# AnnaUshnova/tinyrenderder

Hardware: AMD Instinct MI355X
Metric: triangles/sec (+ Mpixels/sec) at 4096x4096; achieved HBM GB/s vs peak (higher is better)
Workload: dtype f64

## Files before the change

tinyrenderder_amd/api.py:

```python
from __future__ import annotations

import ctypes as C
import os
import sys

import numpy as np

HERE = os.path.dirname(os.path.abspath(__file__))
LIB_PATH = os.path.join(HERE, "libtrgl.so")

FLAT, GOURAUD, PHONG, EYE, CHECKER = 0, 1, 2, 3, 4
VARY = {FLAT: 0, GOURAUD: 3, PHONG: 24, EYE: 24, CHECKER: 0}
SHADER_USER_FIRST, MAX_USER_SHADERS, MAX_USER_VARY = 64, 32, 64
SHADER_MAY_DISCARD = 1
SHADER_READS_DEST = 4
SHADER_NO_DEPTH_WRITE = 8


def shader_flags(may_discard=False, reads_dest=False, depth_write=True) -> int:
    return ((SHADER_MAY_DISCARD if may_discard else 0) | (SHADER_READS_DEST if reads_dest else 0)
            | (0 if depth_write else SHADER_NO_DEPTH_WRITE))
MAX_USER_VERTEX_SHADERS = 32
MEM_HOST, MEM_DEVICE = 0, 1
PHASE_SETUP, PHASE_BIN, PHASE_RASTER, PHASE_TOTAL, PHASE_RASTER_KERNEL = 0, 1, 2, 3, 4
# ... 131 lines not shown
    L.trgl_draw.argtypes = [vp, C.c_int, C.POINTER(Uniforms), C.c_void_p, C.c_void_p, C.c_void_p, C.c_uint64, C.c_int]
    L.trgl_flush.argtypes = [vp]
    L.trgl_flush_begin.argtypes = [vp]
    L.trgl_flush_end.argtypes = [vp]
    L.trgl_sync.argtypes = [vp]
    L.trgl_read_framebuffer.argtypes = [vp, C.c_void_p]
    L.trgl_write_framebuffer.argtypes = [vp, C.c_void_p]
    L.trgl_read_zbuffer.argtypes = [vp, C.c_void_p]
    L.trgl_write_zbuffer.argtypes = [vp, C.c_void_p]
    L.trgl_get_stats.argtypes = [vp, C.POINTER(Stats)]
    L.trgl_reset_stats.argtypes = [vp]
    L.trgl_format_stats.argtypes = [C.POINTER(Stats), C.c_char_p, C.c_size_t]
    for name in ("trgl_framebuffer_device_ptr", "trgl_zbuffer_device_ptr", "trgl_stream"):
        getattr(L, name).argtypes = [vp]; getattr(L, name).restype = C.c_void_p
    L.trgl_set_stream.argtypes = [vp, C.c_void_p, C.c_int]
    L.trgl_set_profiling.argtypes = [vp, C.c_int]
    L.trgl_get_phase_ms.argtypes = [vp, dp, u64p]
    L.trgl_reset_phase_ms.argtypes = [vp]
    L.trgl_get_last_flush_info.argtypes = [vp, u64p, u64p, u64p]
    if hasattr(L, "trgl_debug_read"):
        L.trgl_debug_read.argtypes = [vp, C.c_int, C.c_void_p, C.c_size_t, C.POINTER(C.c_size_t)]
    if hasattr(L, "trgl_debug_binning"):
        L.trgl_debug_binning.argtypes = [vp, C.c_int, C.c_uint32, C.c_uint32, C.POINTER(C.c_int), C.POINTER(C.c_int)]
    L.trgl_selftest_division.argtypes = [vp, C.c_uint64, C.c_uint64, u64p]
    L.trgl_selftest_sampler.argtypes = [vp, C.c_int, C.c_void_p, C.c_uint64, C.c_void_p]
    L.trgl_draw_indexed.argtypes = [vp, C.c_int, C.POINTER(Uniforms), dp, C.c_void_p, C.c_int, C.c_uint64, C.c_void_p, C.c_uint64, C.c_int]
    L.trgl_ssao_defaults.argtypes = [C.POINTER(SsaoParams)]
    L.trgl_ssao_defaults.restype = None
    L.trgl_postprocess.argtypes = [vp, C.POINTER(SsaoParams), C.c_void_p, C.c_void_p, C.c_void_p]
    L.trgl_obj_load.argtypes = [C.c_char_p, C.POINTER(C.POINTER(C.c_double)), u64p, C.POINTER(C.POINTER(C.c_uint32)), u64p]
    L.trgl_obj_free.argtypes = [C.POINTER(C.c_double), C.POINTER(C.c_uint32)]
    L.trgl_obj_free.restype = None
    L.trgl_tga_max_size.argtypes = [C.c_int, C.c_int, C.c_int]
    L.trgl_tga_max_size.restype = C.c_size_t
    L.trgl_tga_encode.argtypes = [C.c_void_p, C.c_int, C.c_int, C.c_int, C.c_int, C.c_int, C.c_void_p, C.POINTER(C.c_size_t)]
    L.trgl_tga_info.argtypes = [C.c_void_p, C.c_size_t, C.POINTER(C.c_int), C.POINTER(C.c_int), C.POINTER(C.c_int)]
    L.trgl_tga_decode.argtypes = [C.c_void_p, C.c_size_t, C.c_void_p]
    L.trgl_gather.argtypes = [vp, C.c_void_p, C.c_int, C.c_int, C.c_int]
    L.trgl_rccl_unique_id.argtypes = [C.c_void_p]
    L.trgl_rccl_comm_create.argtypes = [C.c_void_p, C.c_int, C.c_int, C.c_int, C.POINTER(C.c_void_p)]
    L.trgl_rccl_comm_destroy.argtypes = [C.c_void_p]
    L.trgl_shader_compile.argtypes = [C.c_char_p, C.c_int, C.c_char_p, C.c_size_t]
    L.trgl_register_shader.argtypes = [vp, C.c_char_p, C.c_int, C.POINTER(C.c_int)]
    L.trgl_shader_compile_ex.argtypes = [C.c_char_p, C.c_int, C.c_uint32, C.c_char_p, C.c_size_t]
    L.trgl_register_shader_ex.argtypes = [vp, C.c_char_p, C.c_int, C.c_uint32, C.POINTER(C.c_int)]
    L.trgl_vertex_shader_compile.argtypes = [C.c_char_p, C.c_int, C.c_char_p, C.c_size_t]
# ... 1092 lines not shown
        self._chk(self.L.trgl_reset_phase_ms(self.h))

    def selftest_division(self, samples: int, seed: int = 1) -> int:
        bad = C.c_uint64()
        self._chk(self.L.trgl_selftest_division(self.h, samples, seed, C.byref(bad)))
        return bad.value

    def selftest_sampler(self, slot: int, uv) -> np.ndarray:
        uv = np.ascontiguousarray(uv, np.float64).reshape(-1, 2)
        out = np.zeros((uv.shape[0], 5), np.uint8)
        self._chk(self.L.trgl_selftest_sampler(self.h, slot, uv.ctypes.data, uv.shape[0], out.ctypes.data))
        return out

    def last_flush_info(self):
        a, b, c = C.c_uint64(), C.c_uint64(), C.c_uint64()
        self._chk(self.L.trgl_get_last_flush_info(self.h, C.byref(a), C.byref(b), C.byref(c)))
        return dict(triangles=a.value, pairs=b.value, tiles=c.value)

    def debug_binning(self, mode=None, S=0, G=0):
        d, f = C.c_int(), C.c_int()
        self._chk(self.L.trgl_debug_binning(self.h, -1 if mode is None else mode, S, G, C.byref(d), C.byref(f)))
        return dict(direct=bool(d.value), fell_back=bool(f.value))

    def _debug_read(self, what, dtype):
        need = C.c_size_t()
        self._chk(self.L.trgl_debug_read(self.h, what, None, 0, C.byref(need)))
        out = np.zeros(need.value // np.dtype(dtype).itemsize, dtype)
        if need.value:
            self._chk(self.L.trgl_debug_read(self.h, what, out.ctypes.data, out.nbytes, None))
        return out

    def debug_snapshot(self):
        info = dict(zip(DBG_INFO_FIELDS, (int(v) for v in self._debug_read(DBG_INFO, np.int64))))
        return dict(info=info, recs=self._debug_read(DBG_RECS, TRI_REC), cnt=self._debug_read(DBG_CNT, np.uint32),
                    tilebox=self._debug_read(DBG_TILEBOX, np.uint32).reshape(-1, 2), vals=self._debug_read(DBG_VALS, np.uint32),
                    bmask=self._debug_read(DBG_BMASK, np.uint16), tile_start=self._debug_read(DBG_TILE_START, np.uint32),
                    tile_end=self._debug_read(DBG_TILE_END, np.uint32))
```

tinyrenderder_amd/csrc/kernels_bin.hip:

```cpp
#include <hip/hip_runtime.h>
#include "trgl_device.h"
#include "launch.h"
#include "device_util.h"

namespace {

__device__ __forceinline__ double dmin3(double a, double b, double c) { double m = a; if (b < m) m = b; if (c < m) m = c; return m; }
__device__ __forceinline__ double dmax3(double a, double b, double c) { double m = a; if (m < b) m = b; if (m < c) m = c; return m; }
using trgl_dev::dot4; using trgl_dev::wave_incl_scan; using trgl_dev::block_excl_scan;

__device__ __forceinline__ int wave_min_i(int v) {
    for (int o = 32; o; o >>= 1) { int t = __shfl_xor(v, o); v = t < v ? t : v; }
    return v;
}
__device__ __forceinline__ int wave_max_i(int v) {
    for (int o = 32; o; o >>= 1) { int t = __shfl_xor(v, o); v = t > v ? t : v; }
    return v;
}

__device__ __forceinline__ uint32_t tile_block_mask(uint32_t tx, uint32_t ty, uint32_t qx0, uint32_t qy0, uint32_t qx1, uint32_t qy1) {
    const uint32_t c0 = qx0 > 4 * tx ? qx0 - 4 * tx : 0u, c1 = qx1 < 4 * tx + 3 ? qx1 - 4 * tx : 3u;
    const uint32_t r0 = qy0 > 4 * ty ? qy0 - 4 * ty : 0u, r1 = qy1 < 4 * ty + 3 ? qy1 - 4 * ty : 3u;
    return (((2u << c1) - (1u << c0)) & 0xfu) * 0x1111u & ((0xffffu >> (12 - 4 * r1)) & (0xffffu << (4 * r0)));
}
// ... 417 lines not shown
        for (int o = 1; o < 64; o <<= 1) { const uint32_t t = __shfl_up(inc, o); if (lane >= o) inc += t; }
        if (lane == 63) s_wave[w] = inc;
        __syncthreads();
        uint32_t wbase = 0, tot = 0;
#pragma unroll
        for (int k = 0; k < ROWSCAN_THREADS / 64; ++k) { const uint32_t t = s_wave[k]; if (k < w) wbase += t; tot += t; }
        uint32_t run = running + wbase + inc - sum;
#pragma unroll
        for (int k = 0; k < ROWSCAN_PER; ++k) { if (base + k < nblocks) row[base + k] = run; run += v[k]; }
        running += tot;
        __syncthreads();
    }
    if (threadIdx.x == 0) totals[blockIdx.x] = running;
}

template <int R, int N, class F>
__device__ __forceinline__ void rounds_below(uint32_t part, F& f) {
    if constexpr (R < N) {
        if ((uint32_t)(R * 64) < part) { f(R); rounds_below<R + 1, N>(part, f); }
    }
}

template <int RADIX_WAVES, bool WIDE, bool LAST, bool SEG>
__global__ __launch_bounds__(RADIX_WAVES * 64) void k_radix_scatter(const uint32_t* __restrict__ keys_in, const uint32_t* __restrict__ vals_in,
                                                                 const uint16_t* __restrict__ msk_in,
                                                                 const unsigned long long* __restrict__ pairs_total, uint32_t cap,
                                                                 int shift, int bits, uint32_t nblocks,
                                                                 const uint32_t* __restrict__ base, const uint32_t* __restrict__ totals,
                                                                 uint32_t* __restrict__ keys_out, uint32_t* __restrict__ vals_out,
                                                                 uint16_t* __restrict__ msk_out,
                                                                 uint32_t* __restrict__ tile_start, uint32_t* __restrict__ tile_end, SegIn seg) {
    constexpr int RADIX_THREADS = RADIX_WAVES * 64, RADIX_CHUNK = RADIX_WAVES * RADIX_WAVE_CHUNK;
    static_assert(!(SEG && WIDE), "the direct path sorts 32-bit sort words only");
    __shared__ uint32_t s_off[SEG ? SEG_MAX_GROUP + 1 : 1];
    __shared__ uint32_t s_cnt[RADIX_WAVES][1 << RADIX_MAX_BITS];
    __shared__ uint32_t s_start[1 << RADIX_MAX_BITS];
    __shared__ uint32_t s_gbase[1 << RADIX_MAX_BITS];
    __shared__ uint32_t s_val[RADIX_CHUNK];
    __shared__ uint32_t s_key[RADIX_CHUNK];
    __shared__ uint16_t s_msk[WIDE ? RADIX_CHUNK : 2];
    const int w = threadIdx.x >> 6, lane = threadIdx.x & 63;
    const unsigned long long P64 = *pairs_total;
    const uint32_t P = (P64 > cap || (!SEG && seg.flag && *seg.flag)) ? 0u : (uint32_t)P64;
    if (!SEG && (uint64_t)blockIdx.x * RADIX_CHUNK >= P) return;
    if (SEG) {
        if (*seg.flag || P64 > cap) return;
        const uint32_t b = blockIdx.x * seg.G + lane;
        if (w == 0) {
            const uint32_t c = (lane < seg.G && b < seg.nsetup) ? seg.blk_sums[b] : 0u;
            const uint32_t inc = wave_incl_scan(c);
            if (lane <= SEG_MAX_GROUP) s_off[lane] = inc - c;
        }
    }
    const uint32_t nb = 1u << bits, mask = nb - 1;
    for (uint32_t b = threadIdx.x; b < nb; b += RADIX_THREADS) {
#pragma unroll
        for (int ww = 0; ww < RADIX_WAVES; ++ww) s_cnt[ww][b] = 0;
        s_gbase[b] = base[(size_t)b * nblocks + blockIdx.x];
    }
    if (w == 0) {
        uint32_t tot[4], run = 0;
#pragma unroll
        for (int q = 0; q < 4; ++q) { const uint32_t d = lane * 4 + q; tot[q] = d < nb ? totals[d] : 0; run += tot[q]; }
        uint32_t inc = run;
        for (int o = 1; o < 64; o <<= 1) { const uint32_t t = __shfl_up(inc, o); if (lane >= o) inc += t; }
        uint32_t ex = inc - run;
#pragma unroll
        for (int q = 0; q < 4; ++q) { const uint32_t d = lane * 4 + q; if (d < nb) s_start[d] = ex; ex += tot[q]; }
    }
    __syncthreads();
    for (uint32_t b = threadIdx.x; b < nb; b += RADIX_THREADS) s_gbase[b] += s_start[b];
    __syncthreads();
    const uint64_t cbeg = SEG ? 0 : (uint64_t)blockIdx.x * RADIX_CHUNK;
    uint64_t cend = cbeg + RADIX_CHUNK; if (cend > P) cend = P;
    uint32_t wave_part = RADIX_WAVE_CHUNK;
    if (SEG) {
        cend = (uint32_t)__builtin_amdgcn_readfirstlane((int)s_off[SEG_MAX_GROUP]);
        if (cend > (uint64_t)RADIX_CHUNK || seg.S > SEG_MAX || seg.G > SEG_MAX_GROUP) return;
        wave_part = (((uint32_t)cend + RADIX_THREADS - 1) / RADIX_THREADS) * 64;
    }
    const uint32_t n_chunk = (uint32_t)(cend - cbeg);
    const uint64_t wbeg = cbeg + (uint64_t)w * wave_part;
    const unsigned long long lt = (1ull << lane) - 1ull;

    uint32_t k[RADIX_ROUNDS], v[RADIX_ROUNDS], rk[RADIX_ROUNDS];
    uint16_t mk[WIDE ? RADIX_ROUNDS : 1];
#pragma unroll
    for (int r = 0; r < RADIX_ROUNDS; ++r) {
        const uint64_t p = wbeg + (uint64_t)r * 64 + lane;
        const bool act = p < cend && (!SEG || r * 64 < (int)wave_part);
        if (SEG) {
            const uint32_t lp = (uint32_t)p;
            uint32_t sg = 0;
            if (act) {
#pragma unroll
                for (uint32_t st = SEG_MAX_GROUP / 2; st; st >>= 1) if (lp >= s_off[sg + st]) sg += st;
            }
            const size_t a = (size_t)(blockIdx.x * seg.G + sg) * seg.S + (lp - s_off[sg]);
            k[r] = act ? keys_in[a] : 0; v[r] = act ? vals_in[a] : 0;
        } else {
            k[r] = act ? keys_in[p] : 0; v[r] = act ? vals_in[p] : 0;
            if (WIDE) mk[WIDE ? r : 0] = act ? msk_in[p] : (uint16_t)0;
        }
    }
    auto rank_round = [&](const int r) {
        const bool act = wbeg + (uint64_t)r * 64 + lane < cend;
        const uint32_t dgt = (k[r] >> shift) & mask;
        unsigned long long same = __ballot(act);
        for (int b = 0; b < bits; ++b) {
            const unsigned long long bal = __ballot((dgt >> b) & 1u);
            same &= ((dgt >> b) & 1u) ? bal : ~bal;
        }
        const uint32_t cur = act ? s_cnt[w][dgt] : 0;
        __builtin_amdgcn_wave_barrier();
        const uint32_t r_in = __popcll(same & lt);
        rk[r] = cur + r_in;
        if (act && r_in == 0) s_cnt[w][dgt] = cur + (uint32_t)__popcll(same);
        __builtin_amdgcn_wave_barrier();
    };
    if constexpr (SEG) {
        rounds_below<0, RADIX_ROUNDS>(wave_part, rank_round);
    } else {
#pragma unroll
        for (int r = 0; r < RADIX_ROUNDS; ++r) rank_round(r);
    }
    __syncthreads();
    if (w == 0) {
        uint32_t tot[4], run = 0;
#pragma unroll
        for (int q = 0; q < 4; ++q) {
            const uint32_t d = lane * 4 + q;
            uint32_t t = 0;
            if (d < nb) {
#pragma unroll
                for (int ww = 0; ww < RADIX_WAVES; ++ww) t += s_cnt[ww][d];
            }
            tot[q] = t;
            run += tot[q];
        }
        uint32_t inc = run;
        for (int o = 1; o < 64; o <<= 1) { const uint32_t t = __shfl_up(inc, o); if (lane >= o) inc += t; }
        uint32_t ex = inc - run;
#pragma unroll
        for (int q = 0; q < 4; ++q) { const uint32_t d = lane * 4 + q; if (d < nb) s_start[d] = ex; ex += tot[q]; }
    }
    __syncthreads();
    for (uint32_t d = threadIdx.x; d < nb; d += RADIX_THREADS) {
        uint32_t run = s_start[d];
#pragma unroll
        for (int ww = 0; ww < RADIX_WAVES; ++ww) { const uint32_t c = s_cnt[ww][d]; s_cnt[ww][d] = run; run += c; }
    }
    __syncthreads();
    auto place_round = [&](const int r) {
        if (wbeg + (uint64_t)r * 64 + lane < cend) {
            const uint32_t dgt = (k[r] >> shift) & mask;
            const uint32_t lp = s_cnt[w][dgt] + rk[r];
            s_key[lp] = k[r]; s_val[lp] = v[r];
            if (WIDE) s_msk[lp] = mk[WIDE ? r : 0];
        }
    };
    if constexpr (SEG) {
        rounds_below<0, RADIX_ROUNDS>(wave_part, place_round);
    } else {
#pragma unroll
        for (int r = 0; r < RADIX_ROUNDS; ++r) place_round(r);
    }
    __syncthreads();
    constexpr uint32_t KEY_MASK = WIDE ? 0xffffffffu : 0xffffu;
    for (uint32_t i = threadIdx.x; i < n_chunk; i += RADIX_THREADS) {
        const uint32_t word = s_key[i];
        const uint32_t dgt = (word >> shift) & mask;
        const uint32_t dst = s_gbase[dgt] + (i - s_start[dgt]);
        vals_out[dst] = s_val[i];
        if (!LAST) {
            keys_out[dst] = word;
            if (WIDE) msk_out[dst] = s_msk[i];
        } else {
            msk_out[dst] = WIDE ? s_msk[i] : (uint16_t)(word >> 16);
            const uint32_t key = word & KEY_MASK;
            if (i == 0 || (s_key[i - 1] & KEY_MASK) != key) atomicMin(&tile_start[key], dst);
            if (i + 1 == n_chunk || (s_key[i + 1] & KEY_MASK) != key) atomicMax(&tile_end[key], dst + 1);
        }
    }
}

}

namespace trgl {

uint32_t setup_num_blocks(uint32_t n) { return (n + SETUP_THREADS - 1) / SETUP_THREADS; }

void launch_setup(hipStream_t s, const FrameParams& fp, const DrawDesc& draw, DrawDesc* draws_dev, int draw_idx, uint32_t n,
                  TriRec* recs, TriW* recs_w, uint32_t* cnt, uint2* tilebox, DevStats* stats, uint32_t* blk_sums, uint32_t blk_base,
                  const SegLayout* seg) {
    if (!n) return;
    hipLaunchKernelGGL(k_setup, dim3(setup_num_blocks(n)), dim3(SETUP_THREADS), 0, s, fp, draw, draws_dev, draw_idx, recs, recs_w, cnt, tilebox,
                       stats, blk_sums, blk_base, seg ? seg->keys : nullptr, seg ? seg->vals : nullptr, seg ? seg->S : 0u);
}

void launch_chunk_spine(hipStream_t s, const uint32_t* blk_sums, uint32_t nblk, uint32_t* chunk_off, unsigned long long* total64, unsigned long long* host_copy,
                        uint32_t* tile_bounds, size_t half_words, uint32_t seg_S, uint32_t seg_G, uint32_t seg_chunk, uint32_t* seg_flag,
                        uint32_t* seg_flag_host) {
    hipLaunchKernelGGL(k_chunk_spine, dim3(1), dim3(SPINE_THREADS), 0, s, blk_sums, nblk, chunk_off, total64, host_copy, (uint4*)tile_bounds,
                       (uint32_t)(half_words / 4), seg_S, seg_G, seg_chunk, seg_flag, seg_flag_host);
}

void launch_expand(hipStream_t s, const FrameParams& fp, uint32_t first, uint32_t n, int tiles_x, const uint32_t* cnt, const uint32_t* blk_sums,
                   const uint32_t* chunk_off, uint32_t blk_base, const uint2* tilebox, uint32_t* keys, bool wide, uint32_t* vals, uint16_t* bmask,
                   const unsigned long long* pairs_total, uint32_t cap) {
    if (!n) return;
    if (wide)
        hipLaunchKernelGGL(k_expand<true>, dim3(setup_num_blocks(n)), dim3(SETUP_THREADS), 0, s, fp, first, n, tiles_x, cnt, blk_sums, chunk_off,
                           blk_base, tilebox, keys, vals, bmask, pairs_total, cap);
    else
        hipLaunchKernelGGL(k_expand<false>, dim3(setup_num_blocks(n)), dim3(SETUP_THREADS), 0, s, fp, first, n, tiles_x, cnt, blk_sums, chunk_off,
                           blk_base, tilebox, keys, vals, bmask, pairs_total, cap);
}

static uint32_t radix_waves(uint32_t cap) { return cap >= RADIX_BIG_CAP ? 8u : 4u; }
uint32_t radix_chunk(uint32_t cap) { return radix_waves(cap) * RADIX_WAVE_CHUNK; }
uint32_t radix_num_workers(uint32_t cap) { const uint64_t chunk = radix_chunk(cap); return (uint32_t)((cap + chunk - 1) / chunk); }
uint32_t seg_num_groups(const SegLayout& seg) { return (seg.nsetup + seg.G - 1) / seg.G; }
bool seg_layout_ok(const SegLayout& seg) { return seg.S >= 4 && seg.S <= SEG_MAX && seg.S % 4 == 0 && seg.G >= 1 && seg.G <= SEG_MAX_GROUP; }

template <int WAVES, bool WIDE, bool LAST>
static void radix_pass_t(hipStream_t s, const RadixPass& ps, const unsigned long long* pairs_total, uint32_t cap, uint32_t* hist, uint32_t* scan_tmp,
                         const uint32_t* skip) {
    const uint32_t nblk = radix_num_workers(cap);
    hipLaunchKernelGGL(k_radix_hist, dim3(nblk), dim3(256), 0, s, ps.keys_in, pairs_total, cap, ps.shift, ps.bits, (uint32_t)(WAVES * RADIX_WAVE_CHUNK),
                       nblk, hist, skip);
    hipLaunchKernelGGL(k_radix_scan_rows, dim3(1u << ps.bits), dim3(ROWSCAN_THREADS), 0, s, hist, nblk, scan_tmp);
    hipLaunchKernelGGL((k_radix_scatter<WAVES, WIDE, LAST, false>), dim3(nblk), dim3(WAVES * 64), 0, s, ps.keys_in, ps.vals_in, ps.msk_in, pairs_total, cap,
                       ps.shift, ps.bits, nblk, hist, scan_tmp, ps.keys_out, ps.vals_out, ps.msk_out, ps.tile_start, ps.tile_end, SegIn{ nullptr, skip, 0, 0, 0 });
}
template <int WAVES, bool LAST>
static void radix_pass_seg(hipStream_t s, const RadixPass& ps, const SegLayout& sl, const unsigned long long* pairs_total, uint32_t cap, uint32_t* hist,
                           uint32_t* scan_tmp) {
    const uint32_t nblk = seg_num_groups(sl);
    const SegIn seg{ sl.blk_sums, sl.flag, sl.nsetup, sl.S, sl.G };
    hipLaunchKernelGGL(k_radix_hist_seg, dim3(nblk), dim3(256), 0, s, sl.keys, seg, pairs_total, cap, ps.shift, ps.bits, nblk, hist);
    hipLaunchKernelGGL(k_radix_scan_rows, dim3(1u << ps.bits), dim3(ROWSCAN_THREADS), 0, s, hist, nblk, scan_tmp);
    hipLaunchKernelGGL((k_radix_scatter<WAVES, false, LAST, true>), dim3(nblk), dim3(WAVES * 64), 0, s, sl.keys, sl.vals, ps.msk_in, pairs_total, cap,
                       ps.shift, ps.bits, nblk, hist, scan_tmp, ps.keys_out, ps.vals_out, ps.msk_out, ps.tile_start, ps.tile_end, seg);
}

template <int WAVES>
static void radix_pass_w(hipStream_t s, const RadixPass& ps, bool wide, bool last, const unsigned long long* pairs_total, uint32_t cap,
                         uint32_t* hist, uint32_t* scan_tmp, const SegLayout* seg, const uint32_t* skip) {
    if (seg) { if (last) radix_pass_seg<WAVES, true>(s, ps, *seg, pairs_total, cap, hist, scan_tmp); else radix_pass_seg<WAVES, false>(s, ps, *seg, pairs_total, cap, hist, scan_tmp); }
    else if (wide) { if (last) radix_pass_t<WAVES, true, true>(s, ps, pairs_total, cap, hist, scan_tmp, skip); else radix_pass_t<WAVES, true, false>(s, ps, pairs_total, cap, hist, scan_tmp, skip); }
    else { if (last) radix_pass_t<WAVES, false, true>(s, ps, pairs_total, cap, hist, scan_tmp, skip); else radix_pass_t<WAVES, false, false>(s, ps, pairs_total, cap, hist, scan_tmp, skip); }
}

void launch_radix_pass(hipStream_t s, const RadixPass& ps, bool wide, bool last, const unsigned long long* pairs_total, uint32_t cap,
                       uint32_t* hist, uint32_t* scan_tmp, const SegLayout* seg, const uint32_t* skip) {
    if (!cap || (seg && (wide || !seg->nsetup))) return;
    if (radix_waves(cap) == 8) radix_pass_w<8>(s, ps, wide, last, pairs_total, cap, hist, scan_tmp, seg, skip);
    else radix_pass_w<4>(s, ps, wide, last, pairs_total, cap, hist, scan_tmp, seg, skip);
}

}
```

tinyrenderder_amd/csrc/launch.h:

```cpp
#pragma once
#include <hip/hip_runtime.h>
#include "trgl_device.h"
#include "clip_core.h"
#include "work_items.h"

namespace trgl {

struct SegLayout { uint32_t* keys; uint32_t* vals; const uint32_t* blk_sums; const uint32_t* flag; uint32_t nsetup, S, G; };
bool seg_layout_ok(const SegLayout& seg);
uint32_t seg_num_groups(const SegLayout& seg);

uint32_t setup_num_blocks(uint32_t n);
void launch_setup(hipStream_t s, const FrameParams& fp, const DrawDesc& draw, DrawDesc* draws_dev, int draw_idx, uint32_t n,
                  TriRec* recs, TriW* recs_w, uint32_t* cnt, uint2* tilebox, DevStats* stats, uint32_t* blk_sums, uint32_t blk_base,
                  const SegLayout* seg);
void launch_chunk_spine(hipStream_t s, const uint32_t* blk_sums, uint32_t nblk, uint32_t* chunk_off, unsigned long long* total64, unsigned long long* host_copy,
                        uint32_t* tile_bounds, size_t half_words, uint32_t seg_S, uint32_t seg_G, uint32_t seg_chunk, uint32_t* seg_flag,
                        uint32_t* seg_flag_host);


void launch_expand(hipStream_t s, const FrameParams& fp, uint32_t first, uint32_t n, int tiles_x, const uint32_t* cnt, const uint32_t* blk_sums,
                   const uint32_t* chunk_off, uint32_t blk_base, const uint2* tilebox, uint32_t* keys, bool wide, uint32_t* vals, uint16_t* bmask,
                   const unsigned long long* pairs_total, uint32_t cap);

uint32_t radix_num_workers(uint32_t cap);
uint32_t radix_chunk(uint32_t cap);
struct RadixPass {
    const uint32_t* keys_in; const uint32_t* vals_in; const uint16_t* msk_in;
    uint32_t* keys_out; uint32_t* vals_out; uint16_t* msk_out;
    uint32_t* tile_start; uint32_t* tile_end;
    int shift, bits;
};
void launch_radix_pass(hipStream_t s, const RadixPass& ps, bool wide, bool last, const unsigned long long* pairs_total, uint32_t cap,
                       uint32_t* hist, uint32_t* scan_tmp, const SegLayout* seg = nullptr, const uint32_t* skip = nullptr);

uint32_t owned_tiles(const FrameParams& fp);
uint32_t raster_max_items(const FrameParams& fp);
void launch_make_items(hipStream_t s, const FrameParams& fp, int tiles, const uint32_t* tile_start, const uint32_t* tile_end, uint4* items,
                       uint32_t* n_items, TriRec* recs);
void launch_fold_stats(hipStream_t s, DevStats* stats, uint32_t* n_items, const unsigned long long* item_stats);
struct UserShade { hipFunction_t fn; int kind; };
void launch_raster(hipStream_t s, const FrameParams& fp, int kind, bool all_well_scaled, const TriRec* recs, const TriW* recs_w,
                   const uint32_t* vals, const uint16_t* bmask,
                   const uint32_t* tile_start, const uint32_t* tile_end, const DrawDesc* draws,
                   const DevTexture* tex, DevStats* stats, uint32_t max_items, uint4* items,
                   uint32_t* n_items, unsigned long long* item_stats, bool builtin_shade, const UserShade* user, int n_user,
                   hipFunction_t user_raster,
                   hipEvent_t ev_before = nullptr, hipEvent_t ev_after = nullptr);

void launch_vertex_stage(hipStream_t s, const double mv[16], const double proj[16], const double* vertices, int stride,
                         const uint32_t* indices, uint32_t nfaces, double* clip, double* vary);
void launch_zimage(hipStream_t s, const double* zb, int W, int H, unsigned long long* keys2, uint8_t* out);
void launch_ssao(hipStream_t s, const double* zb, int W, int H, const double* dir_x, const double* dir_y, int ndir, int steps,
                 double radius, double threshold, double intensity, uint8_t* out);
void launch_composite(hipStream_t s, const uint8_t* fb, int bpp, const uint8_t* ao, int W, int H, uint8_t* out);

struct BoundsPartial { double v[6]; unsigned long long i[6]; };
// ... 77 lines not shown
```

tinyrenderder_amd/csrc/trgl_api.cpp:

```cpp
#include <algorithm>
#include <cstring>

#include "trgl_ctx.h"
#include "user_shaders.h"

static size_t pair_capacity(size_t need) {
    const size_t ncap = (headroom(need) + 3) & ~size_t(3);
    return ncap > 0xffffe000ull ? 0xffffe000ull : ncap;
}

int trgl::fail(trgl_ctx* c, int code, const std::string& msg) { if (c) c->err = msg; else set_global_error(msg); return code; }

static int reset_dev_stats(trgl_ctx* c) {
    DevStats s;
    s.fragments = 0;
    s.zmin_key = zkey(std::numeric_limits<double>::infinity());
    s.zmax_key = zkey(-std::numeric_limits<double>::infinity());
    s.min_x = INT32_MAX; s.min_y = INT32_MAX; s.max_x = INT32_MIN; s.max_y = INT32_MIN;
    s.pairs_total = 0; s.literal_tris = 0; s.large_tris = 0;
    s.zero_pos_key = s.zero_neg_key = TRGL_ZERO_KEY_EMPTY;
    s.zero_locked = 0; s.zero_sign = 0;
    for (int k = 0; k < 16; ++k) s.dbg[k] = 0;
    *c->stats_pinned = s;
    HIPCHK(c, hipMemcpyAsync(c->stats_dev.p, c->stats_pinned, sizeof(DevStats), hipMemcpyHostToDevice, c->stream));
// ... 248 lines not shown
static int queue_binning(trgl_ctx* c, const FrameParams& fp, uint32_t cap, int* cur_out, const SegLayout* seg) {
    hipStream_t s = c->stream;
    const size_t ntiles = (size_t)c->tiles_x * c->tiles_y;
    const unsigned long long* pairs_dev = &c->stats_dev.p->pairs_total;
    int r;
    uint32_t blk_base = 0;
    const bool wide = ntiles > 65536;
    for (auto& d : c->draws) {
        if (seg) break;
        launch_expand(s, fp, d.first, d.n, c->tiles_x, c->cnt.p, c->blk_sums.p, c->chunk_off.p, blk_base, c->tilebox.p, c->keys[0].p, wide, c->vals[0].p,
                      c->bmask[0].p, pairs_dev, cap);
        blk_base += setup_num_blocks(d.n);
    }
    int key_bits = 1; while ((size_t(1) << key_bits) < ntiles) ++key_bits;
    int passes = (key_bits + 7) / 8;
    int bits_per = (key_bits + passes - 1) / passes;
    size_t hist_need = ((size_t)std::max(radix_num_workers(cap), seg ? seg_num_groups(*seg) : 0u) << bits_per) + 16;
    if ((r = c->hist.grow(c, hist_need))) return r;
    if ((r = c->scan_tmp.grow(c, 256 + 16))) return r;
    int cur = 0;
    for (int ps = 0; ps < passes; ++ps) {
        const RadixPass rp{ c->keys[cur].p, c->vals[cur].p, c->bmask[cur].p, c->keys[cur ^ 1].p, c->vals[cur ^ 1].p, c->bmask[cur ^ 1].p,
                            c->tile_start.p, c->tile_end(), ps * bits_per, bits_per };
        launch_radix_pass(s, rp, wide, ps == passes - 1, pairs_dev, cap, c->hist.p, c->scan_tmp.p, ps == 0 ? seg : nullptr,
                          (seg && ps > 0) ? seg->flag : nullptr);
        cur ^= 1;
    }
    *cur_out = cur;
    return TRGL_OK;
}

static int grow_pairs(trgl_ctx* c, size_t need) {
    const size_t ncap = pair_capacity(need);
    int r;
    for (int k = 0; k < 2; ++k)
        if ((r = c->keys[k].grow(c, need, ncap)) || (r = c->vals[k].grow(c, need, ncap)) || (r = c->bmask[k].grow(c, need, ncap))) return r;
    return TRGL_OK;
}

static bool seg_sizes(double avg, uint32_t chunk, uint32_t* S, uint32_t* G) {
    if (avg < 1.0) avg = 1.0;
    const uint64_t s = ((uint64_t)(avg * 1.5) + 128 + 63) & ~uint64_t(63);
    uint64_t g = (uint64_t)(0.9 * chunk / avg);
    if (g > 16) g = 16;
    if (s > 4096 || g < 2) return false;
    *S = (uint32_t)s; *G = (uint32_t)g;
    return true;
}
// ... 298 lines not shown
    case 6: src = c->tile_end(); need = ntiles * sizeof(uint32_t); break;
    default: need = sizeof(info); break;
    }
    if (needed) *needed = need;
    if (!dst) return TRGL_OK;
    if (bytes < need) return fail(c, TRGL_E_INVALID, "trgl_debug_read: destination too small");
    if (what == 7) { std::memcpy(dst, info, sizeof(info)); return TRGL_OK; }
    HIPCHK(c, hipStreamSynchronize(c->stream));
    if (need) HIPCHK(c, hipMemcpy(dst, src, need, hipMemcpyDeviceToHost));
    return TRGL_OK;
}

extern "C" int trgl_debug_binning(trgl_ctx* c, int mode, uint32_t S, uint32_t G, int* last_direct, int* last_fell_back) {
    CHKCTX(c);
    if (mode < -1 || mode > 2) return fail(c, TRGL_E_INVALID, "trgl_debug_binning: mode is -1 (report only), 0 (automatic), 1 (k_expand) or 2 (direct)");
    if (mode == 2 && !seg_layout_ok(SegLayout{ nullptr, nullptr, nullptr, nullptr, 0, S, G }))
        return fail(c, TRGL_E_INVALID, "trgl_debug_binning: S is a multiple of 4 in 4..4096, G in 1..16");
    if (mode >= 0) { c->bin_mode = mode; c->bin_S = mode == 2 ? S : 0; c->bin_G = mode == 2 ? G : 0; c->seg_hold = false; }
    if (last_direct) *last_direct = c->snap.rp.direct;
    if (last_fell_back) *last_fell_back = c->snap.rp.fell_back;
    return TRGL_OK;
}

int trgl_get_last_flush_info(trgl_ctx* c, uint64_t* triangles, uint64_t* pairs, uint64_t* tiles) {
    if (!c) return TRGL_E_INVALID;
    if (triangles) *triangles = c->snap.rp.N;
    if (pairs) *pairs = c->snap.P;
    if (tiles) *tiles = (uint64_t)c->tiles_x * c->tiles_y;
    return TRGL_OK;
}

}
```

tinyrenderder_amd/csrc/trgl_ctx.h:

```cpp
#pragma once
#include <hip/hip_runtime.h>

#include <limits>
#include <string>
#include <vector>

#include "../../include/trgl.h"
#include "launch.h"
#include "trgl_device.h"

namespace trgl {
struct StageChunk { char* base; size_t cap, used; };

inline size_t headroom(size_t need) { return need + need / 4 + 1024; }
template <class T> struct DevBuf {
    T* p = nullptr;
    size_t cap = 0;
    DevBuf() = default;
    DevBuf(const DevBuf&) = delete;
    ~DevBuf() { if (p) (void)hipFree(p); }
    int alloc(trgl_ctx* c, size_t n);
    int grow(trgl_ctx* c, size_t need, size_t ncap) { return need <= cap ? TRGL_OK : alloc(c, ncap); }
    int grow(trgl_ctx* c, size_t need) { return grow(c, need, headroom(need)); }
    int release(trgl_ctx* c);
// ... 33 lines not shown
    DevBuf<TriRec> recs; DevBuf<TriW> recs_w; DevBuf<uint32_t> cnt; DevBuf<uint2> tilebox;
    PendingRaster rp;
    hipEvent_t ev_pairs = nullptr;
    DevBuf<uint32_t> idbuf;
    DevBuf<BoundsPartial> bounds_scratch;
    DevBuf<uint8_t> mesh_scratch;
    DevBuf<double> zsnap[TRGL_MAX_Z_SNAPSHOTS];
    DevBuf<float> blur_weights; DevBuf<uint8_t> blur_tmp; int blur_radius = 0;
    float* blur_w_pinned = nullptr; size_t blur_w_pinned_cap = 0; hipEvent_t ev_blur_w = nullptr;
    DevBuf<uint32_t> clip_scratch;
    DevBuf<uint8_t> shadow_tmp;
    DevBuf<double> occl_levels, occl_boxes; DevBuf<uint8_t> occl_codes;
    DevBuf<uint32_t> inst_scratch, inst_list; DevBuf<double> inst_mv;
    DevBuf<uint8_t> order_scratch;
    DevBuf<uint8_t> pp_out;
    DevBuf<uint32_t> blk_sums;
    DevBuf<uint32_t> chunk_off;
    DevBuf<uint32_t> keys[2], vals[2]; DevBuf<uint16_t> bmask[2];
    DevBuf<uint32_t> hist, scan_tmp;
    DevBuf<uint32_t> seg_keys, seg_vals, seg_flag;
    uint32_t* seg_flag_pinned = nullptr;
    int bin_mode = 0; uint32_t bin_S = 0, bin_G = 0;
    bool seg_hold = false;
    uint64_t rule_pairs = 0, rule_nblk = 0;
    DevBuf<uint32_t> tile_start;
    DevBuf<uint4> items; DevBuf<uint32_t> n_items;
    DevBuf<unsigned long long> item_stats;
    DevBuf<DrawDesc> draws_dev;
    DevBuf<DevStats> stats_dev;
    DevStats* stats_pinned = nullptr;

    uint64_t triangles_total = 0;
    Snapshot snap;

    bool profiling = false, events_pending = false;
    hipEvent_t ev[6] = { nullptr, nullptr, nullptr, nullptr, nullptr, nullptr };
    double phase_ms[TRGL_NUM_PHASES] = { 0, 0, 0, 0, 0 };
    uint64_t flushes_timed = 0;

    std::vector<UserKind> user;
    std::vector<UserVertex> vertex;

    std::string err;

    size_t bounds_half() const { return ((size_t)tiles_x * tiles_y + 3) & ~size_t(3); }
    uint32_t* tile_end() const { return tile_start.p + bounds_half(); }
// ... 54 lines not shown
```

Baseline: 4.208 billion.

## Make radix scatter persistent with next-chunk prefetch and LDS match-table ranking

The radix scatter kernel now launches at most as many blocks as can be resident, sized by an occupancy query, and loops over chunks in grid-stride fashion. Loads for the next chunk are interleaved with the LDS placement of the current one, so global load latency can overlap with work. Per-digit ranking inside a wave switches from a bit-by-bit ballot loop to wave-scope atomic ORs into a per-wave match table kept in the key staging buffer, and launch bounds now request a minimum occupancy. This adds loop complexity, extra register pressure from double-buffered rounds, and a debug hook to cap the grid size.

Result: faster. 4.291 billion, median of 6 (+2.0%).

```diff
diff --git a/tinyrenderder_amd/api.py b/tinyrenderder_amd/api.py
--- a/tinyrenderder_amd/api.py
+++ b/tinyrenderder_amd/api.py
@@ -177,6 +177,8 @@
         L.trgl_debug_read.argtypes = [vp, C.c_int, C.c_void_p, C.c_size_t, C.POINTER(C.c_size_t)]
     if hasattr(L, "trgl_debug_binning"):
         L.trgl_debug_binning.argtypes = [vp, C.c_int, C.c_uint32, C.c_uint32, C.POINTER(C.c_int), C.POINTER(C.c_int)]
+    if hasattr(L, "trgl_debug_radix_blocks"):
+        L.trgl_debug_radix_blocks.argtypes = [vp, C.c_uint32, C.POINTER(C.c_uint32), C.POINTER(C.c_uint32)]
     L.trgl_selftest_division.argtypes = [vp, C.c_uint64, C.c_uint64, u64p]
     L.trgl_selftest_sampler.argtypes = [vp, C.c_int, C.c_void_p, C.c_uint64, C.c_void_p]
     L.trgl_draw_indexed.argtypes = [vp, C.c_int, C.POINTER(Uniforms), dp, C.c_void_p, C.c_int, C.c_uint64, C.c_void_p, C.c_uint64, C.c_int]
@@ -1315,6 +1317,13 @@
         self._chk(self.L.trgl_debug_binning(self.h, -1 if mode is None else mode, S, G, C.byref(d), C.byref(f)))
         return dict(direct=bool(d.value), fell_back=bool(f.value))
 
+    def debug_radix_blocks(self, n=None):
+        if n is not None:
+            self._radix_blocks = int(n)
+        a, b = C.c_uint32(), C.c_uint32()
+        self._chk(self.L.trgl_debug_radix_blocks(self.h, getattr(self, "_radix_blocks", 0), C.byref(a), C.byref(b)))
+        return dict(first=a.value, last=b.value)
+
     def _debug_read(self, what, dtype):
         need = C.c_size_t()
         self._chk(self.L.trgl_debug_read(self.h, what, None, 0, C.byref(need)))
diff --git a/tinyrenderder_amd/csrc/kernels_bin.hip b/tinyrenderder_amd/csrc/kernels_bin.hip
--- a/tinyrenderder_amd/csrc/kernels_bin.hip
+++ b/tinyrenderder_amd/csrc/kernels_bin.hip
@@ -1,4 +1,5 @@
 #include <hip/hip_runtime.h>
+#include <algorithm>
 #include "trgl_device.h"
 #include "launch.h"
 #include "device_util.h"
@@ -463,7 +464,7 @@
 }
 
 template <int RADIX_WAVES, bool WIDE, bool LAST, bool SEG>
-__global__ __launch_bounds__(RADIX_WAVES * 64) void k_radix_scatter(const uint32_t* __restrict__ keys_in, const uint32_t* __restrict__ vals_in,
+__global__ __launch_bounds__(RADIX_WAVES * 64, WIDE ? 2 : 4) void k_radix_scatter(const uint32_t* __restrict__ keys_in, const uint32_t* __restrict__ vals_in,
                                                                  const uint16_t* __restrict__ msk_in,
                                                                  const unsigned long long* __restrict__ pairs_total, uint32_t cap,
                                                                  int shift, int bits, uint32_t nblocks,
@@ -477,29 +478,32 @@
     __shared__ uint32_t s_cnt[RADIX_WAVES][1 << RADIX_MAX_BITS];
     __shared__ uint32_t s_start[1 << RADIX_MAX_BITS];
     __shared__ uint32_t s_gbase[1 << RADIX_MAX_BITS];
+    __shared__ uint32_t s_tot[1 << RADIX_MAX_BITS];
     __shared__ uint32_t s_val[RADIX_CHUNK];
-    __shared__ uint32_t s_key[RADIX_CHUNK];
+    __shared__ __attribute__((aligned(16))) uint32_t s_key[RADIX_CHUNK];
     __shared__ uint16_t s_msk[WIDE ? RADIX_CHUNK : 2];
-    const int w = threadIdx.x >> 6, lane = threadIdx.x & 63;
+    const int w = __builtin_amdgcn_readfirstlane((int)(threadIdx.x >> 6)), lane = threadIdx.x & 63;
     const unsigned long long P64 = *pairs_total;
     const uint32_t P = (P64 > cap || (!SEG && seg.flag && *seg.flag)) ? 0u : (uint32_t)P64;
-    if (!SEG && (uint64_t)blockIdx.x * RADIX_CHUNK >= P) return;
+    uint32_t nchunks = nblocks;
     if (SEG) {
-        if (*seg.flag || P64 > cap) return;
-        const uint32_t b = blockIdx.x * seg.G + lane;
-        if (w == 0) {
-            const uint32_t c = (lane < seg.G && b < seg.nsetup) ? seg.blk_sums[b] : 0u;
-            const uint32_t inc = wave_incl_scan(c);
-            if (lane <= SEG_MAX_GROUP) s_off[lane] = inc - c;
-        }
-    }
+        if (*seg.flag || P64 > cap || seg.S > SEG_MAX || seg.G > SEG_MAX_GROUP) return;
+    } else {
+        nchunks = min(nblocks, (uint32_t)(((uint64_t)P + RADIX_CHUNK - 1) / RADIX_CHUNK));
+    }
+    uint32_t chunk = blockIdx.x;
+    if (chunk >= nchunks) return;
     const uint32_t nb = 1u << bits, mask = nb - 1;
-    for (uint32_t b = threadIdx.x; b < nb; b += RADIX_THREADS) {
-#pragma unroll
-        for (int ww = 0; ww < RADIX_WAVES; ++ww) s_cnt[ww][b] = 0;
-        s_gbase[b] = base[(size_t)b * nblocks + blockIdx.x];
-    }
+    auto put_offsets = [&](const uint32_t c) {
+        const uint32_t inc = wave_incl_scan(c);
+        if (lane <= SEG_MAX_GROUP) s_off[lane] = inc - c;
+    };
+    auto group_count = [&](const uint32_t c) {
+        const uint32_t b = c * seg.G + lane;
+        return (lane < seg.G && b < seg.nsetup) ? seg.blk_sums[b] : 0u;
+    };
     if (w == 0) {
+        if (SEG) put_offsets(group_count(chunk));
         uint32_t tot[4], run = 0;
 #pragma unroll
         for (int q = 0; q < 4; ++q) { const uint32_t d = lane * 4 + q; tot[q] = d < nb ? totals[d] : 0; run += tot[q]; }
@@ -507,56 +511,74 @@
         for (int o = 1; o < 64; o <<= 1) { const uint32_t t = __shfl_up(inc, o); if (lane >= o) inc += t; }
         uint32_t ex = inc - run;
 #pragma unroll
-        for (int q = 0; q < 4; ++q) { const uint32_t d = lane * 4 + q; if (d < nb) s_start[d] = ex; ex += tot[q]; }
-    }
-    __syncthreads();
-    for (uint32_t b = threadIdx.x; b < nb; b += RADIX_THREADS) s_gbase[b] += s_start[b];
-    __syncthreads();
-    const uint64_t cbeg = SEG ? 0 : (uint64_t)blockIdx.x * RADIX_CHUNK;
-    uint64_t cend = cbeg + RADIX_CHUNK; if (cend > P) cend = P;
-    uint32_t wave_part = RADIX_WAVE_CHUNK;
-    if (SEG) {
-        cend = (uint32_t)__builtin_amdgcn_readfirstlane((int)s_off[SEG_MAX_GROUP]);
-        if (cend > (uint64_t)RADIX_CHUNK || seg.S > SEG_MAX || seg.G > SEG_MAX_GROUP) return;
-        wave_part = (((uint32_t)cend + RADIX_THREADS - 1) / RADIX_THREADS) * 64;
-    }
-    const uint32_t n_chunk = (uint32_t)(cend - cbeg);
-    const uint64_t wbeg = cbeg + (uint64_t)w * wave_part;
+        for (int q = 0; q < 4; ++q) { const uint32_t d = lane * 4 + q; if (d < nb) s_tot[d] = ex; ex += tot[q]; }
+    }
+    __syncthreads();
+    struct Span { uint32_t n, part; };
+    auto span_of = [&](const uint32_t c) {
+        Span sp;
+        if (SEG) {
+            sp.n = (uint32_t)__builtin_amdgcn_readfirstlane((int)s_off[SEG_MAX_GROUP]);
+            sp.part = ((sp.n + RADIX_THREADS - 1) / RADIX_THREADS) * 64;
+        } else {
+            const uint64_t cbeg = (uint64_t)c * RADIX_CHUNK;
+            sp.n = (uint32_t)min((uint64_t)RADIX_CHUNK, (uint64_t)P - cbeg);
+            sp.part = RADIX_WAVE_CHUNK;
+        }
+        return sp;
+    };
+    Span cur = span_of(chunk);
+    if (SEG && cur.n > (uint32_t)RADIX_CHUNK) return;
     const unsigned long long lt = (1ull << lane) - 1ull;
 
+    static_assert(RADIX_WAVE_CHUNK * sizeof(uint32_t) >= (sizeof(unsigned long long) << RADIX_MAX_BITS), "a match table per wave in s_key");
+    unsigned long long* const match = reinterpret_cast<unsigned long long*>(s_key) + (size_t)w * (RADIX_WAVE_CHUNK / 2);
     uint32_t k[RADIX_ROUNDS], v[RADIX_ROUNDS], rk[RADIX_ROUNDS];
     uint16_t mk[WIDE ? RADIX_ROUNDS : 1];
-#pragma unroll
-    for (int r = 0; r < RADIX_ROUNDS; ++r) {
-        const uint64_t p = wbeg + (uint64_t)r * 64 + lane;
-        const bool act = p < cend && (!SEG || r * 64 < (int)wave_part);
+    auto load_round = [&](const int r, const uint32_t c, const Span& sp) {
+        const uint32_t q0 = (uint32_t)w * sp.part + lane, q = q0 + (uint32_t)r * 64;
+        const bool act = (int)q0 < (int)sp.n - r * 64 && (!SEG || (uint32_t)(r * 64) < sp.part);
         if (SEG) {
-            const uint32_t lp = (uint32_t)p;
             uint32_t sg = 0;
             if (act) {
 #pragma unroll
-                for (uint32_t st = SEG_MAX_GROUP / 2; st; st >>= 1) if (lp >= s_off[sg + st]) sg += st;
-            }
-            const size_t a = (size_t)(blockIdx.x * seg.G + sg) * seg.S + (lp - s_off[sg]);
-            k[r] = act ? keys_in[a] : 0; v[r] = act ? vals_in[a] : 0;
+                for (uint32_t st = SEG_MAX_GROUP / 2; st; st >>= 1) if (q >= s_off[sg + st]) sg += st;
+            }
+            const size_t group = (size_t)c * seg.G * seg.S;
+            const uint32_t a = sg * seg.S + (q - s_off[sg]);
+            k[r] = act ? (keys_in + group)[a] : 0; v[r] = act ? (vals_in + group)[a] : 0;
         } else {
-            k[r] = act ? keys_in[p] : 0; v[r] = act ? vals_in[p] : 0;
-            if (WIDE) mk[WIDE ? r : 0] = act ? msk_in[p] : (uint16_t)0;
-        }
-    }
+            const size_t cbeg = (size_t)c * RADIX_CHUNK;
+            k[r] = act ? (keys_in + cbeg)[q] : 0; v[r] = act ? (vals_in + cbeg)[q] : 0;
+            if (WIDE) mk[WIDE ? r : 0] = act ? (msk_in + cbeg)[q] : (uint16_t)0;
+        }
+    };
+#pragma unroll
+    for (int r = 0; r < RADIX_ROUNDS; ++r) load_round(r, chunk, cur);
+
+    for (;;) {
+    const uint32_t next = chunk + gridDim.x;
+    bool more = next < nchunks;
+    const uint32_t wave_part = cur.part, n_chunk = cur.n;
+    const int pos0 = (int)((uint32_t)w * wave_part + lane);
+    const uint32_t gb = threadIdx.x < nb ? base[(size_t)threadIdx.x * nblocks + chunk] : 0u;
+    uint32_t next_count = 0;
+    if (SEG && w == 0 && more) next_count = group_count(next);
+    for (uint32_t d = lane; d < nb; d += 64) { s_cnt[w][d] = 0; match[d] = 0ull; }
+    __builtin_amdgcn_wave_barrier();
     auto rank_round = [&](const int r) {
-        const bool act = wbeg + (uint64_t)r * 64 + lane < cend;
+        const bool act = pos0 < (int)n_chunk - r * 64;
         const uint32_t dgt = (k[r] >> shift) & mask;
-        unsigned long long same = __ballot(act);
-        for (int b = 0; b < bits; ++b) {
-            const unsigned long long bal = __ballot((dgt >> b) & 1u);
-            same &= ((dgt >> b) & 1u) ? bal : ~bal;
-        }
+        unsigned long long* const slot = match + dgt;
+        if (act) __hip_atomic_fetch_or(slot, lt + 1ull, __ATOMIC_RELAXED, __HIP_MEMORY_SCOPE_WAVEFRONT);
+        __builtin_amdgcn_wave_barrier();
+        const unsigned long long same = act ? __hip_atomic_load(slot, __ATOMIC_RELAXED, __HIP_MEMORY_SCOPE_WAVEFRONT) : 0ull;
         const uint32_t cur = act ? s_cnt[w][dgt] : 0;
         __builtin_amdgcn_wave_barrier();
         const uint32_t r_in = __popcll(same & lt);
         rk[r] = cur + r_in;
-        if (act && r_in == 0) s_cnt[w][dgt] = cur + (uint32_t)__popcll(same);
+        asm volatile("" : "+v"(rk[r]));
+        if (act && r_in == 0) { s_cnt[w][dgt] = cur + (uint32_t)__popcll(same); *slot = 0ull; }
         __builtin_amdgcn_wave_barrier();
     };
     if constexpr (SEG) {
@@ -566,7 +588,9 @@
         for (int r = 0; r < RADIX_ROUNDS; ++r) rank_round(r);
     }
     __syncthreads();
+    if (threadIdx.x < nb) s_gbase[threadIdx.x] = gb + s_tot[threadIdx.x];
     if (w == 0) {
+        if (SEG && more) put_offsets(next_count);
         uint32_t tot[4], run = 0;
 #pragma unroll
         for (int q = 0; q < 4; ++q) {
@@ -591,20 +615,24 @@
 #pragma unroll
         for (int ww = 0; ww < RADIX_WAVES; ++ww) { const uint32_t c = s_cnt[ww][d]; s_cnt[ww][d] = run; run += c; }
     }
+    Span nxt = cur;
+    if (more) {
+        nxt = span_of(next);
+        if (SEG && nxt.n > (uint32_t)RADIX_CHUNK) more = false;
+    }
     __syncthreads();
     auto place_round = [&](const int r) {
-        if (wbeg + (uint64_t)r * 64 + lane < cend) {
+        if (pos0 < (int)n_chunk - r * 64) {
             const uint32_t dgt = (k[r] >> shift) & mask;
             const uint32_t lp = s_cnt[w][dgt] + rk[r];
             s_key[lp] = k[r]; s_val[lp] = v[r];
             if (WIDE) s_msk[lp] = mk[WIDE ? r : 0];
         }
     };
-    if constexpr (SEG) {
-        rounds_below<0, RADIX_ROUNDS>(wave_part, place_round);
-    } else {
-#pragma unroll
-        for (int r = 0; r < RADIX_ROUNDS; ++r) place_round(r);
+#pragma unroll
+    for (int r = 0; r < RADIX_ROUNDS; ++r) {
+        if (!SEG || (uint32_t)(r * 64) < wave_part) place_round(r);
+        if (more && (!SEG || (uint32_t)(r * 64) < nxt.part)) load_round(r, next, nxt);
     }
     __syncthreads();
     constexpr uint32_t KEY_MASK = WIDE ? 0xffffffffu : 0xffffu;
@@ -623,6 +651,10 @@
             if (i + 1 == n_chunk || (s_key[i + 1] & KEY_MASK) != key) atomicMax(&tile_end[key], dst + 1);
         }
     }
+    if (!more) break;
+    chunk = next; cur = nxt;
+    __syncthreads();
+    }
 }
 
 }
@@ -664,40 +696,60 @@
 uint32_t seg_num_groups(const SegLayout& seg) { return (seg.nsetup + seg.G - 1) / seg.G; }
 bool seg_layout_ok(const SegLayout& seg) { return seg.S >= 4 && seg.S <= SEG_MAX && seg.S % 4 == 0 && seg.G >= 1 && seg.G <= SEG_MAX_GROUP; }
 
+template <int WAVES, bool WIDE, bool LAST, bool SEG>
+static uint32_t scatter_grid(uint32_t chunks, uint32_t max_blocks) {
+    thread_local int for_dev = -1;
+    thread_local uint32_t resident = 0;
+    int dev = 0;
+    if (hipGetDevice(&dev) != hipSuccess) dev = 0;
+    if (dev != for_dev) {
+        int per_cu = 0, cus = 0;
+        if (hipOccupancyMaxActiveBlocksPerMultiprocessor(&per_cu, k_radix_scatter<WAVES, WIDE, LAST, SEG>, WAVES * 64, 0) != hipSuccess || per_cu < 1) per_cu = 1;
+        if (hipDeviceGetAttribute(&cus, hipDeviceAttributeMultiprocessorCount, dev) != hipSuccess || cus < 1) cus = 1;
+        resident = (uint32_t)per_cu * (uint32_t)cus;
+        for_dev = dev;
+    }
+    uint32_t g = std::min(chunks, resident);
+    if (max_blocks) g = std::min(g, max_blocks);
+    return std::max(g, 1u);
+}
+
 template <int WAVES, bool WIDE, bool LAST>
-static void radix_pass_t(hipStream_t s, const RadixPass& ps, const unsigned long long* pairs_total, uint32_t cap, uint32_t* hist, uint32_t* scan_tmp,
-                         const uint32_t* skip) {
-    const uint32_t nblk = radix_num_workers(cap);
+static uint32_t radix_pass_t(hipStream_t s, const RadixPass& ps, const unsigned long long* pairs_total, uint32_t cap, uint32_t* hist, uint32_t* scan_tmp,
+                             const uint32_t* skip, uint32_t max_blocks) {
+    const uint32_t nblk = radix_num_workers(cap), grid = scatter_grid<WAVES, WIDE, LAST, false>(nblk, max_blocks);
     hipLaunchKernelGGL(k_radix_hist, dim3(nblk), dim3(256), 0, s, ps.keys_in, pairs_total, cap, ps.shift, ps.bits, (uint32_t)(WAVES * RADIX_WAVE_CHUNK),
                        nblk, hist, skip);
     hipLaunchKernelGGL(k_radix_scan_rows, dim3(1u << ps.bits), dim3(ROWSCAN_THREADS), 0, s, hist, nblk, scan_tmp);
-    hipLaunchKernelGGL((k_radix_scatter<WAVES, WIDE, LAST, false>), dim3(nblk), dim3(WAVES * 64), 0, s, ps.keys_in, ps.vals_in, ps.msk_in, pairs_total, cap,
+    hipLaunchKernelGGL((k_radix_scatter<WAVES, WIDE, LAST, false>), dim3(grid), dim3(WAVES * 64), 0, s, ps.keys_in, ps.vals_in, ps.msk_in, pairs_total, cap,
                        ps.shift, ps.bits, nblk, hist, scan_tmp, ps.keys_out, ps.vals_out, ps.msk_out, ps.tile_start, ps.tile_end, SegIn{ nullptr, skip, 0, 0, 0 });
+    return grid;
 }
 template <int WAVES, bool LAST>
-static void radix_pass_seg(hipStream_t s, const RadixPass& ps, const SegLayout& sl, const unsigned long long* pairs_total, uint32_t cap, uint32_t* hist,
-                           uint32_t* scan_tmp) {
-    const uint32_t nblk = seg_num_groups(sl);
+static uint32_t radix_pass_seg(hipStream_t s, const RadixPass& ps, const SegLayout& sl, const unsigned long long* pairs_total, uint32_t cap, uint32_t* hist,
+                               uint32_t* scan_tmp, uint32_t max_blocks) {
+    const uint32_t nblk = seg_num_groups(sl), grid = scatter_grid<WAVES, false, LAST, true>(nblk, max_blocks);
     const SegIn seg{ sl.blk_sums, sl.flag, sl.nsetup, sl.S, sl.G };
     hipLaunchKernelGGL(k_radix_hist_seg, dim3(nblk), dim3(256), 0, s, sl.keys, seg, pairs_total, cap, ps.shift, ps.bits, nblk, hist);
     hipLaunchKernelGGL(k_radix_scan_rows, dim3(1u << ps.bits), dim3(ROWSCAN_THREADS), 0, s, hist, nblk, scan_tmp);
-    hipLaunchKernelGGL((k_radix_scatter<WAVES, false, LAST, true>), dim3(nblk), dim3(WAVES * 64), 0, s, sl.keys, sl.vals, ps.msk_in, pairs_total, cap,
+    hipLaunchKernelGGL((k_radix_scatter<WAVES, false, LAST, true>), dim3(grid), dim3(WAVES * 64), 0, s, sl.keys, sl.vals, ps.msk_in, pairs_total, cap,
                        ps.shift, ps.bits, nblk, hist, scan_tmp, ps.keys_out, ps.vals_out, ps.msk_out, ps.tile_start, ps.tile_end, seg);
+    return grid;
 }
 
 template <int WAVES>
-static void radix_pass_w(hipStream_t s, const RadixPass& ps, bool wide, bool last, const unsigned long long* pairs_total, uint32_t cap,
-                         uint32_t* hist, uint32_t* scan_tmp, const SegLayout* seg, const uint32_t* skip) {
-    if (seg) { if (last) radix_pass_seg<WAVES, true>(s, ps, *seg, pairs_total, cap, hist, scan_tmp); else radix_pass_seg<WAVES, false>(s, ps, *seg, pairs_total, cap, hist, scan_tmp); }
-    else if (wide) { if (last) radix_pass_t<WAVES, true, true>(s, ps, pairs_total, cap, hist, scan_tmp, skip); else radix_pass_t<WAVES, true, false>(s, ps, pairs_total, cap, hist, scan_tmp, skip); }
-    else { if (last) radix_pass_t<WAVES, false, true>(s, ps, pairs_total, cap, hist, scan_tmp, skip); else radix_pass_t<WAVES, false, false>(s, ps, pairs_total, cap, hist, scan_tmp, skip); }
-}
-
-void launch_radix_pass(hipStream_t s, const RadixPass& ps, bool wide, bool last, const unsigned long long* pairs_total, uint32_t cap,
-                       uint32_t* hist, uint32_t* scan_tmp, const SegLayout* seg, const uint32_t* skip) {
-    if (!cap || (seg && (wide || !seg->nsetup))) return;
-    if (radix_waves(cap) == 8) radix_pass_w<8>(s, ps, wide, last, pairs_total, cap, hist, scan_tmp, seg, skip);
-    else radix_pass_w<4>(s, ps, wide, last, pairs_total, cap, hist, scan_tmp, seg, skip);
-}
-
-}
+static uint32_t radix_pass_w(hipStream_t s, const RadixPass& ps, bool wide, bool last, const unsigned long long* pairs_total, uint32_t cap,
+                             uint32_t* hist, uint32_t* scan_tmp, const SegLayout* seg, const uint32_t* skip, uint32_t mb) {
+    if (seg) return last ? radix_pass_seg<WAVES, true>(s, ps, *seg, pairs_total, cap, hist, scan_tmp, mb) : radix_pass_seg<WAVES, false>(s, ps, *seg, pairs_total, cap, hist, scan_tmp, mb);
+    if (wide) return last ? radix_pass_t<WAVES, true, true>(s, ps, pairs_total, cap, hist, scan_tmp, skip, mb) : radix_pass_t<WAVES, true, false>(s, ps, pairs_total, cap, hist, scan_tmp, skip, mb);
+    return last ? radix_pass_t<WAVES, false, true>(s, ps, pairs_total, cap, hist, scan_tmp, skip, mb) : radix_pass_t<WAVES, false, false>(s, ps, pairs_total, cap, hist, scan_tmp, skip, mb);
+}
+
+uint32_t launch_radix_pass(hipStream_t s, const RadixPass& ps, bool wide, bool last, const unsigned long long* pairs_total, uint32_t cap,
+                           uint32_t* hist, uint32_t* scan_tmp, const SegLayout* seg, const uint32_t* skip, uint32_t max_blocks) {
+    if (!cap || (seg && (wide || !seg->nsetup))) return 0;
+    if (radix_waves(cap) == 8) return radix_pass_w<8>(s, ps, wide, last, pairs_total, cap, hist, scan_tmp, seg, skip, max_blocks);
+    return radix_pass_w<4>(s, ps, wide, last, pairs_total, cap, hist, scan_tmp, seg, skip, max_blocks);
+}
+
+}
diff --git a/tinyrenderder_amd/csrc/launch.h b/tinyrenderder_amd/csrc/launch.h
--- a/tinyrenderder_amd/csrc/launch.h
+++ b/tinyrenderder_amd/csrc/launch.h
@@ -31,8 +31,9 @@
     uint32_t* tile_start; uint32_t* tile_end;
     int shift, bits;
 };
-void launch_radix_pass(hipStream_t s, const RadixPass& ps, bool wide, bool last, const unsigned long long* pairs_total, uint32_t cap,
-                       uint32_t* hist, uint32_t* scan_tmp, const SegLayout* seg = nullptr, const uint32_t* skip = nullptr);
+uint32_t launch_radix_pass(hipStream_t s, const RadixPass& ps, bool wide, bool last, const unsigned long long* pairs_total, uint32_t cap,
+                           uint32_t* hist, uint32_t* scan_tmp, const SegLayout* seg = nullptr, const uint32_t* skip = nullptr,
+                           uint32_t max_blocks = 0);
 
 uint32_t owned_tiles(const FrameParams& fp);
 uint32_t raster_max_items(const FrameParams& fp);
diff --git a/tinyrenderder_amd/csrc/trgl_api.cpp b/tinyrenderder_amd/csrc/trgl_api.cpp
--- a/tinyrenderder_amd/csrc/trgl_api.cpp
+++ b/tinyrenderder_amd/csrc/trgl_api.cpp
@@ -294,8 +294,10 @@
     for (int ps = 0; ps < passes; ++ps) {
         const RadixPass rp{ c->keys[cur].p, c->vals[cur].p, c->bmask[cur].p, c->keys[cur ^ 1].p, c->vals[cur ^ 1].p, c->bmask[cur ^ 1].p,
                             c->tile_start.p, c->tile_end(), ps * bits_per, bits_per };
-        launch_radix_pass(s, rp, wide, ps == passes - 1, pairs_dev, cap, c->hist.p, c->scan_tmp.p, ps == 0 ? seg : nullptr,
-                          (seg && ps > 0) ? seg->flag : nullptr);
+        const uint32_t grid = launch_radix_pass(s, rp, wide, ps == passes - 1, pairs_dev, cap, c->hist.p, c->scan_tmp.p, ps == 0 ? seg : nullptr,
+                                                (seg && ps > 0) ? seg->flag : nullptr, c->radix_max_blocks);
+        if (ps == 0) c->radix_used[0] = grid;
+        if (ps == passes - 1) c->radix_used[1] = grid;
         cur ^= 1;
     }
     *cur_out = cur;
@@ -640,6 +642,14 @@
     return TRGL_OK;
 }
 
+extern "C" int trgl_debug_radix_blocks(trgl_ctx* c, uint32_t max_blocks, uint32_t* used_first, uint32_t* used_last) {
+    CHKCTX(c);
+    c->radix_max_blocks = max_blocks;
+    if (used_first) *used_first = c->radix_used[0];
+    if (used_last) *used_last = c->radix_used[1];
+    return TRGL_OK;
+}
+
 int trgl_get_last_flush_info(trgl_ctx* c, uint64_t* triangles, uint64_t* pairs, uint64_t* tiles) {
     if (!c) return TRGL_E_INVALID;
     if (triangles) *triangles = c->snap.rp.N;
diff --git a/tinyrenderder_amd/csrc/trgl_ctx.h b/tinyrenderder_amd/csrc/trgl_ctx.h
--- a/tinyrenderder_amd/csrc/trgl_ctx.h
+++ b/tinyrenderder_amd/csrc/trgl_ctx.h
@@ -79,6 +79,7 @@
     uint32_t* seg_flag_pinned = nullptr;
     int bin_mode = 0; uint32_t bin_S = 0, bin_G = 0;
     bool seg_hold = false;
+    uint32_t radix_max_blocks = 0, radix_used[2] = { 0, 0 };
     uint64_t rule_pairs = 0, rule_nblk = 0;
     DevBuf<uint32_t> tile_start;
     DevBuf<uint4> items; DevBuf<uint32_t> n_items;
```
